# XiaokunSun/SemanticHuman

Hardware: AMD Instinct MI355X
Metric: training meshes/sec at 6890 verts, batch=64 (higher is better)
Workload: dtype f32

## Files before the change

semantichuman_amd/csrc/linear.hip:

```cpp
#include "sh_bf16.h"
#include "sh_adam.h"

#include <type_traits>

namespace {

constexpr int LT = 64;
constexpr int LK = 32;
constexpr int LTHREADS = 256;

struct SGParams {
    const float* a; long a_sm, a_sr;
    const float* b; long b_sn, b_sr;
    float* c; long c_sm, c_sn;
    const float* bias;
    float* slab;
    int M, N, R;
    int rchunk, nsplit, n_mtiles, n_ntiles;
    int a_mode, b_mode;
};

__device__ __forceinline__ void sg_load(const float* base, long s_row, long s_r, int mode, int row0, int nrows, int r0, int rend,
                                        int tid, f32x4 (&reg)[2], unsigned& mask) {
    mask = 0;
// ... 242 lines not shown
#pragma unroll
                for (int mt = 0; mt < MT; ++mt) acc[mt][nt] = __builtin_amdgcn_mfma_f32_16x16x4f32(w4[nt][t], x4[mt][t], acc[mt][nt], 0, 0, 0);
    };
    auto step = [&](int s, auto J) {
        constexpr int j = decltype(J)::value;
        load(s + LS_DEPTH - 1, xa[(j + LS_DEPTH - 1) % LS_DEPTH], wb[(j + LS_DEPTH - 1) % LS_DEPTH]);
        __builtin_amdgcn_sched_barrier(0);
        mma(xa[j], wb[j]);
    };
    if (nsteps > 0) {
#pragma unroll
        for (int d = 0; d < LS_DEPTH - 1; ++d) load(d, xa[d], wb[d]);
        for (int s = 0; s < nsteps; s += LS_DEPTH)
            if (ls_run_steps<0, LS_DEPTH>(s, nsteps, step)) break;
    }
#pragma unroll
    for (int mt = 0; mt < MT; ++mt) {
        const int m = 16 * mt + lr;
        if (m >= p.M) continue;
#pragma unroll
        for (int nt = 0; nt < 4; ++nt) {
            const int n = n0 + 16 * nt + 4 * kq;
            f32x4 v = acc[mt][nt];
            if (p.nsplit > 1) {
                *reinterpret_cast<f32x4*>(p.slab + ((long)sp * p.M + m) * p.N + n) = v;
            } else {
                if (p.bias) v += *reinterpret_cast<const f32x4*>(p.bias + n);
                *reinterpret_cast<f32x4*>(p.out + (long)m * p.N + n) = v;
            }
        }
    }
}

constexpr int LFD_STAGE = 40 * 1024, LFD_LDS = 3 * LFD_STAGE;
__device__ __forceinline__ f32x4 lin_x3_mma(const bf16x8 ah, const bf16x8 am, const bf16x8 al, const bf16x8 bh, const bf16x8 bm, const bf16x8 bl,
                                            f32x4 c) {
    c = __builtin_amdgcn_mfma_f32_16x16x32_bf16(al, bh, c, 0, 0, 0);
    c = __builtin_amdgcn_mfma_f32_16x16x32_bf16(ah, bl, c, 0, 0, 0);
    c = __builtin_amdgcn_mfma_f32_16x16x32_bf16(am, bm, c, 0, 0, 0);
    c = __builtin_amdgcn_mfma_f32_16x16x32_bf16(am, bh, c, 0, 0, 0);
    c = __builtin_amdgcn_mfma_f32_16x16x32_bf16(ah, bm, c, 0, 0, 0);
    return __builtin_amdgcn_mfma_f32_16x16x32_bf16(ah, bh, c, 0, 0, 0);
}
struct LinX3 { bf16x8 h, m, l; };
__device__ __forceinline__ LinX3 lin_split(const f32x4 a, const f32x4 b) {
    u32x4 h, m, l;
    sh_split3(a, b, h, m, l);
    return LinX3{__builtin_bit_cast(bf16x8, h), __builtin_bit_cast(bf16x8, m), __builtin_bit_cast(bf16x8, l)};
}

template <int MT, bool X3 = false>
__global__ __launch_bounds__(LTHREADS) void linear_fwd_dma_kernel(const LSParams p) {
    extern __shared__ __attribute__((aligned(16))) char smem[];
    const int lane = threadIdx.x & 63;
    const int wave = __builtin_amdgcn_readfirstlane((int)(threadIdx.x >> 6));
    const int item = sh_xcd_remap(blockIdx.x, gridDim.x) * 4 + wave;
    const int ng = item % p.groups, sp = item / p.groups;
    const int n0 = ng * 64, k_begin = sp * p.range;
    const int nst = (min(p.K, k_begin + p.range) - k_begin) >> 5;
    const int m_lo = 64 * (int)blockIdx.y, m_n = min(64, p.M - m_lo);
    const float* pa = p.a + (long)m_lo * p.K;
    const int lr = lane & 15, kq = lane >> 4;
    typedef __attribute__((address_space(3))) char* lptr_t;
    const unsigned lds0 = __builtin_amdgcn_readfirstlane((unsigned)(uintptr_t)(lptr_t)smem);
    auto dma16 = [](const void* gsrc, unsigned lds_dst) {
        asm volatile("s_mov_b32 m0, %1\n\ts_nop 0\n\tglobal_load_lds_dwordx4 %0, off" : : "v"(gsrc), "s"(lds_dst) : "memory", "m0");
    };
    const int drow = lane >> 3;
    const float* wsrc[8];
    const float* xsrc[2];
#pragma unroll
    for (int q = 0; q < 8; ++q) {
        const int r = 8 * q + drow, piece = (lane & 7) ^ ((r >> 1) & 7);
        wsrc[q] = p.w + (long)(n0 + r) * p.K + k_begin + 4 * piece;
    }
#pragma unroll
    for (int j = 0; j < 2; ++j) {
        const int r = 8 * (2 * wave + j) + drow, piece = (lane & 7) ^ ((r >> 1) & 7);
        xsrc[j] = pa + (long)min(r, m_n - 1) * p.K + k_begin + 4 * piece;
    }
    auto issue = [&](int st) {
        const unsigned slot = lds0 + (unsigned)((st % 3) * LFD_STAGE);
        const int off = 32 * (st < nst ? st : nst - 1);
#pragma unroll
        for (int j = 0; j < 2; ++j) dma16(xsrc[j] + off, slot + (unsigned)((2 * wave + j) * 1024));
#pragma unroll
        for (int q = 0; q < 8; ++q) dma16(wsrc[q] + off, slot + (unsigned)(8192 + wave * 8192 + q * 1024));
    };
    f32x4 acc[MT][4];
#pragma unroll
    for (int mt = 0; mt < MT; ++mt)
#pragma unroll
        for (int nt = 0; nt < 4; ++nt) acc[mt][nt] = (f32x4){0.f, 0.f, 0.f, 0.f};
    const int sw = (lr >> 1) & 7;
    const int foff0 = lr * 128 + ((kq ^ sw) << 4), foff1 = lr * 128 + (((4 + kq) ^ sw) << 4);
    if (nst > 0) {
        issue(0);
        issue(1);
        for (int st = 0; st < nst; ++st) {
            asm volatile("s_waitcnt vmcnt(10)" ::: "memory");
            __syncthreads();
            issue(st + 2);
            const char* sl = smem + (st % 3) * LFD_STAGE;
            const char* wl = sl + 8192 + wave * 8192;
            if constexpr (X3) {
                LinX3 xs[MT];
#pragma unroll
                for (int mt = 0; mt < MT; ++mt)
                    xs[mt] = lin_split(*reinterpret_cast<const f32x4*>(sl + mt * 2048 + foff0), *reinterpret_cast<const f32x4*>(sl + mt * 2048 + foff1));
#pragma unroll
                for (int nt = 0; nt < 4; ++nt) {
                    const LinX3 ws = lin_split(*reinterpret_cast<const f32x4*>(wl + nt * 2048 + foff0), *reinterpret_cast<const f32x4*>(wl + nt * 2048 + foff1));
#pragma unroll
                    for (int mt = 0; mt < MT; ++mt) acc[mt][nt] = lin_x3_mma(ws.h, ws.m, ws.l, xs[mt].h, xs[mt].m, xs[mt].l, acc[mt][nt]);
                }
                continue;
            }
#pragma unroll
            for (int h = 0; h < 2; ++h) {
                const int fo = h == 0 ? foff0 : foff1;
                f32x4 w4[4], x4[MT];
#pragma unroll
                for (int nt = 0; nt < 4; ++nt) w4[nt] = *reinterpret_cast<const f32x4*>(wl + nt * 2048 + fo);
#pragma unroll
                for (int mt = 0; mt < MT; ++mt) x4[mt] = *reinterpret_cast<const f32x4*>(sl + mt * 2048 + fo);
#pragma unroll
                for (int t = 0; t < 4; ++t)
#pragma unroll
                    for (int nt = 0; nt < 4; ++nt)
#pragma unroll
                        for (int mt = 0; mt < MT; ++mt) acc[mt][nt] = __builtin_amdgcn_mfma_f32_16x16x4f32(w4[nt][t], x4[mt][t], acc[mt][nt], 0, 0, 0);
            }
        }
        asm volatile("s_waitcnt vmcnt(0)" ::: "memory");
    }
#pragma unroll
    for (int mt = 0; mt < MT; ++mt) {
        if (16 * mt + lr >= m_n) continue;
        const int m = m_lo + 16 * mt + lr;
#pragma unroll
        for (int nt = 0; nt < 4; ++nt) {
            const int n = n0 + 16 * nt + 4 * kq;
            f32x4 v = acc[mt][nt];
            if (p.nsplit > 1) {
                *reinterpret_cast<f32x4*>(p.slab + ((long)sp * p.M + m) * p.N + n) = v;
            } else {
                if (p.bias) v += *reinterpret_cast<const f32x4*>(p.bias + n);
                *reinterpret_cast<f32x4*>(p.out + (long)m * p.N + n) = v;
            }
        }
    }
}

constexpr int LFW_WAVES = 8;
__global__ __launch_bounds__(LFW_WAVES * 64) void linear_fwd_wide_x3_kernel(const LSParams p) {
    extern __shared__ __attribute__((aligned(16))) char smem[];
    u32x4* Wl = reinterpret_cast<u32x4*>(smem);
    const int lane = threadIdx.x & 63, wave = sh_wave_id();
    const int n0 = sh_xcd_remap(blockIdx.x, gridDim.x) * 64;
    const int nks = p.K >> 5;
    const int lr = lane & 15, kq = lane >> 4;
    for (int f = wave; f < nks * 4; f += LFW_WAVES) {
        const int ks = f >> 2, nt = f & 3;
        const float* src = p.w + (long)(n0 + 16 * nt + lr) * p.K + 32 * ks + 8 * kq;
        u32x4 h, m, l;
        sh_split3(*reinterpret_cast<const f32x4*>(src), *reinterpret_cast<const f32x4*>(src + 4), h, m, l);
        u32x4* d = Wl + (long)f * 192 + lane;
        d[0] = h; d[64] = m; d[128] = l;
    }
    __syncthreads();
    for (int m0 = 16 * wave; m0 < p.M; m0 += 16 * LFW_WAVES) {
        const int mrow = m0 + lr;
        const float* xr = p.a + (long)min(mrow, p.M - 1) * p.K + 8 * kq;
        f32x4 acc[4];
#pragma unroll
        for (int nt = 0; nt < 4; ++nt) acc[nt] = (f32x4){0.f, 0.f, 0.f, 0.f};
        f32x4 xa = *reinterpret_cast<const f32x4*>(xr), xb = *reinterpret_cast<const f32x4*>(xr + 4);
        for (int ks = 0; ks < nks; ++ks) {
            const int kn = ks + 1 < nks ? ks + 1 : ks;
            const f32x4 na = *reinterpret_cast<const f32x4*>(xr + 32 * kn), nb = *reinterpret_cast<const f32x4*>(xr + 32 * kn + 4);
            const LinX3 xs = lin_split(xa, xb);
            const u32x4* wk = Wl + (long)ks * 4 * 192 + lane;
#pragma unroll
            for (int nt = 0; nt < 4; ++nt) {
                const u32x4 r0 = wk[nt * 192], r1 = wk[nt * 192 + 64], r2 = wk[nt * 192 + 128];
                acc[nt] = lin_x3_mma(__builtin_bit_cast(bf16x8, r0), __builtin_bit_cast(bf16x8, r1), __builtin_bit_cast(bf16x8, r2), xs.h, xs.m,
                                     xs.l, acc[nt]);
            }
            xa = na; xb = nb;
        }
        if (mrow < p.M) {
#pragma unroll
            for (int nt = 0; nt < 4; ++nt) {
                const int n = n0 + 16 * nt + 4 * kq;
                f32x4 v = acc[nt];
                if (p.bias) v += *reinterpret_cast<const f32x4*>(p.bias + n);
                *reinterpret_cast<f32x4*>(p.out + (long)mrow * p.N + n) = v;
            }
        }
    }
}

template <int MT>
__global__ __launch_bounds__(LTHREADS) void linear_bwd_data_stream_kernel(const LSParams p) {
    const int lane = threadIdx.x & 63, wave = sh_wave_id();
    const int item = sh_xcd_remap(blockIdx.x, gridDim.x) * 4 + wave;
    if (item >= p.groups * p.nsplit) return;
    const int kg = item % p.groups, sp = item / p.groups;
    const int k0 = kg * 64, n_begin = sp * p.range;
    const int nsteps = (min(p.N, n_begin + p.range) - n_begin) >> 4;
    const int la = lane & 15, rr = lane >> 4;
    const float* drow[MT];
#pragma unroll
    for (int mt = 0; mt < MT; ++mt) drow[mt] = p.a + (long)min(16 * mt + la, p.M - 1) * p.N + n_begin + 4 * rr;
    const float* wbase = p.w + (long)(n_begin + 4 * rr) * p.K + k0 + 4 * la;
    f32x4 dq[LS_DEPTH][MT], wq[LS_DEPTH][4], acc[4][MT];
#pragma unroll
    for (int t = 0; t < 4; ++t)
#pragma unroll
        for (int mt = 0; mt < MT; ++mt) acc[t][mt] = (f32x4){0.f, 0.f, 0.f, 0.f};
    auto load = [&](int s, f32x4 (&d4)[MT], f32x4 (&w4)[4]) {
        const int nb = 16 * (s < nsteps ? s : nsteps - 1);
#pragma unroll
        for (int mt = 0; mt < MT; ++mt) d4[mt] = *reinterpret_cast<const f32x4*>(drow[mt] + nb);
#pragma unroll
        for (int e = 0; e < 4; ++e) w4[e] = __builtin_nontemporal_load(reinterpret_cast<const f32x4*>(wbase + (long)(nb + e) * p.K));
    };
    auto mma = [&](const f32x4 (&d4)[MT], const f32x4 (&w4)[4]) {
#pragma unroll
        for (int e = 0; e < 4; ++e)
#pragma unroll
            for (int t = 0; t < 4; ++t)
#pragma unroll
                for (int mt = 0; mt < MT; ++mt) acc[t][mt] = __builtin_amdgcn_mfma_f32_16x16x4f32(w4[e][t], d4[mt][e], acc[t][mt], 0, 0, 0);
    };
    auto step = [&](int s, auto J) {
        constexpr int j = decltype(J)::value;
        load(s + LS_DEPTH - 1, dq[(j + LS_DEPTH - 1) % LS_DEPTH], wq[(j + LS_DEPTH - 1) % LS_DEPTH]);
        __builtin_amdgcn_sched_barrier(0);
        mma(dq[j], wq[j]);
    };
    if (nsteps > 0) {
#pragma unroll
        for (int d = 0; d < LS_DEPTH - 1; ++d) load(d, dq[d], wq[d]);
        for (int s = 0; s < nsteps; s += LS_DEPTH)
            if (ls_run_steps<0, LS_DEPTH>(s, nsteps, step)) break;
    }
#pragma unroll
    for (int mt = 0; mt < MT; ++mt) {
        const int m = 16 * mt + la;
        if (m >= p.M) continue;
        float* dst = (p.nsplit > 1 ? p.slab + ((long)sp * p.M + m) * p.K : p.out + (long)m * p.K) + k0 + 16 * rr;
#pragma unroll
        for (int jj = 0; jj < 4; ++jj)
            *reinterpret_cast<f32x4*>(dst + 4 * jj) = (f32x4){acc[0][mt][jj], acc[1][mt][jj], acc[2][mt][jj], acc[3][mt][jj]};
    }
}

template <int MT>
__global__ __launch_bounds__(LTHREADS) void linear_bwd_data_x3_kernel(const LSParams p) {
    const int lane = threadIdx.x & 63, wave = sh_wave_id();
    const int item = sh_xcd_remap(blockIdx.x, gridDim.x) * 4 + wave;
    if (item >= p.groups * p.nsplit) return;
    const int kg = item % p.groups, sp = item / p.groups;
    const int k0 = kg * 64, n_begin = sp * p.range;
    const int nsteps = (min(p.N, n_begin + p.range) - n_begin) >> 5;
    const int la = lane & 15, rr = lane >> 4;
    const float* drow[MT];
#pragma unroll
    for (int mt = 0; mt < MT; ++mt) drow[mt] = p.a + (long)min(16 * mt + la, p.M - 1) * p.N + n_begin + 4 * rr;
    const float* wbase = p.w + (long)(n_begin + 4 * rr) * p.K + k0 + 4 * la;
    f32x4 dq[2][MT][2], wq[2][8], acc[4][MT];
#pragma unroll
    for (int t = 0; t < 4; ++t)
#pragma unroll
        for (int mt = 0; mt < MT; ++mt) acc[t][mt] = (f32x4){0.f, 0.f, 0.f, 0.f};
    auto load = [&](int s, f32x4 (&d4)[MT][2], f32x4 (&w4)[8]) {
        const int nb = 32 * (s < nsteps ? s : nsteps - 1);
#pragma unroll
        for (int mt = 0; mt < MT; ++mt) {
            d4[mt][0] = *reinterpret_cast<const f32x4*>(drow[mt] + nb);
            d4[mt][1] = *reinterpret_cast<const f32x4*>(drow[mt] + nb + 16);
        }
#pragma unroll
        for (int j = 0; j < 8; ++j)
            w4[j] = __builtin_nontemporal_load(reinterpret_cast<const f32x4*>(wbase + (long)(nb + (j & 3) + 16 * (j >> 2)) * p.K));
    };
    auto mma = [&](const f32x4 (&d4)[MT][2], const f32x4 (&w4)[8]) {
        LinX3 ds[MT];
#pragma unroll
        for (int mt = 0; mt < MT; ++mt) ds[mt] = lin_split(d4[mt][0], d4[mt][1]);
#pragma unroll
        for (int t = 0; t < 4; ++t) {
            const LinX3 ws = lin_split((f32x4){w4[0][t], w4[1][t], w4[2][t], w4[3][t]}, (f32x4){w4[4][t], w4[5][t], w4[6][t], w4[7][t]});
#pragma unroll
            for (int mt = 0; mt < MT; ++mt) acc[t][mt] = lin_x3_mma(ws.h, ws.m, ws.l, ds[mt].h, ds[mt].m, ds[mt].l, acc[t][mt]);
        }
    };
    if (nsteps > 0) {
        load(0, dq[0], wq[0]);
        for (int s = 0; s < nsteps; s += 2) {
            load(s + 1, dq[1], wq[1]);
            __builtin_amdgcn_sched_barrier(0);
            mma(dq[0], wq[0]);
            if (s + 1 >= nsteps) break;
            load(s + 2, dq[0], wq[0]);
            __builtin_amdgcn_sched_barrier(0);
            mma(dq[1], wq[1]);
        }
    }
#pragma unroll
    for (int mt = 0; mt < MT; ++mt) {
        const int m = 16 * mt + la;
        if (m >= p.M) continue;
        float* dst = (p.nsplit > 1 ? p.slab + ((long)sp * p.M + m) * p.K : p.out + (long)m * p.K) + k0 + 16 * rr;
#pragma unroll
        for (int jj = 0; jj < 4; ++jj)
            *reinterpret_cast<f32x4*>(dst + 4 * jj) = (f32x4){acc[0][mt][jj], acc[1][mt][jj], acc[2][mt][jj], acc[3][mt][jj]};
    }
}

__global__ __launch_bounds__(LTHREADS) void linear_bwd_wgt_stream_kernel(const LSParams p) {
    const int lane = threadIdx.x & 63, wave = sh_wave_id();
    const int item = sh_xcd_remap(blockIdx.x, gridDim.x) * 4 + wave;
    const int ktiles = p.K >> 6;
    if (item >= (p.N >> 6) * ktiles) return;
    const int kt = item % ktiles, ntile = item / ktiles;
    const int n0 = ntile * 64, k0 = kt * 64;
    const int la = lane & 15, rr = lane >> 4;
    const int nsteps = (p.M + 3) >> 2;
    f32x4 acc[4][4];
#pragma unroll
    for (int a = 0; a < 4; ++a)
#pragma unroll
        for (int b = 0; b < 4; ++b) acc[a][b] = (f32x4){0.f, 0.f, 0.f, 0.f};
    f32x4 dq[4], xq[4];
    auto load = [&](int s, f32x4& d4, f32x4& x4) {
        s = s < nsteps ? s : nsteps - 1;
        const int m = 4 * s + rr;
        const int mc = m < p.M ? m : p.M - 1;
        d4 = *reinterpret_cast<const f32x4*>(p.a + (long)mc * p.N + n0 + 4 * la);
        x4 = *reinterpret_cast<const f32x4*>(p.w + (long)mc * p.K + k0 + 4 * la);
        if (m >= p.M) d4 = (f32x4){0.f, 0.f, 0.f, 0.f};
    };
    const bool own_bias = kt == 0 && p.dbias != nullptr;
    f32x4 bsum = {0.f, 0.f, 0.f, 0.f};
    auto mma = [&](const f32x4& d4, const f32x4& x4) {
#pragma unroll
        for (int tn = 0; tn < 4; ++tn)
#pragma unroll
            for (int tk = 0; tk < 4; ++tk) acc[tn][tk] = __builtin_amdgcn_mfma_f32_16x16x4f32(d4[tn], x4[tk], acc[tn][tk], 0, 0, 0);
        if (own_bias) bsum += d4;
    };
    load(0, dq[0], xq[0]); load(1, dq[1], xq[1]); load(2, dq[2], xq[2]);
    for (int s = 0; s < nsteps; s += 4) {
        load(s + 3, dq[3], xq[3]); __builtin_amdgcn_sched_barrier(0); mma(dq[0], xq[0]);
        if (s + 1 >= nsteps) break;
        load(s + 4, dq[0], xq[0]); __builtin_amdgcn_sched_barrier(0); mma(dq[1], xq[1]);
        if (s + 2 >= nsteps) break;
        load(s + 5, dq[1], xq[1]); __builtin_amdgcn_sched_barrier(0); mma(dq[2], xq[2]);
        if (s + 3 >= nsteps) break;
        load(s + 6, dq[2], xq[2]); __builtin_amdgcn_sched_barrier(0); mma(dq[3], xq[3]);
    }
    if (own_bias) {
#pragma unroll
        for (int j = 0; j < 4; ++j) {
            float v = bsum[j];
            v += __shfl_xor(v, 16, 64);
            v += __shfl_xor(v, 32, 64);
            bsum[j] = v;
        }
        if (rr == 0) *reinterpret_cast<f32x4*>(p.dbias + n0 + 4 * la) = bsum;
    }
#pragma unroll
    for (int tn = 0; tn < 4; ++tn)
#pragma unroll
        for (int jj = 0; jj < 4; ++jj) {
            float* dst = p.out + (long)(n0 + 16 * rr + 4 * jj + tn) * p.K + k0 + 4 * la;
            __builtin_nontemporal_store((f32x4){acc[tn][0][jj], acc[tn][1][jj], acc[tn][2][jj], acc[tn][3][jj]}, reinterpret_cast<f32x4*>(dst));
        }
}

constexpr int LWD_TILE = 16 * 1024, LWD_LDS = 5 * LWD_TILE;
template <bool X3 = false, bool ADAM = false, bool A16 = false, bool W16 = false>
__global__ __launch_bounds__(LTHREADS) __attribute__((amdgpu_waves_per_eu((X3 || ADAM) ? 2 : 1, (X3 || ADAM) ? 2 : 8)))
void linear_bwd_wgt_dma_kernel(const LSParams p) {
    extern __shared__ __attribute__((aligned(16))) char smem[];
    const int lane = threadIdx.x & 63;
    const int wave = __builtin_amdgcn_readfirstlane((int)(threadIdx.x >> 6));
    const int ktiles = p.K >> 6, kgroups = (ktiles + 3) >> 2;
    const int item = sh_xcd_remap(blockIdx.x, gridDim.x);
    const int kg = item % kgroups, ntile = item / kgroups;
    const int kt = kg * 4 + wave;
    const bool active = kt < ktiles;
    const int n0 = ntile * 64, k0 = (active ? kt : 0) * 64;
    const int la = lane & 15, rr = lane >> 4;
    const int nsteps = (p.M + 3) >> 2;
    typedef __attribute__((address_space(3))) char* lptr_t;
    const unsigned lds0 = __builtin_amdgcn_readfirstlane((unsigned)(uintptr_t)(lptr_t)smem);
    auto dma16 = [](const void* gsrc, unsigned lds_dst) {
        asm volatile("s_mov_b32 m0, %1\n\ts_nop 0\n\tglobal_load_lds_dwordx4 %0, off" : : "v"(gsrc), "s"(lds_dst) : "memory", "m0");
    };
    const int piece = (lane & 15) ^ ((lane >> 4) << 2);
    auto stage16 = [&](const __bf16* src, long ld, int col0, int row, int j, char* tile) {
        const bf16x8 v = *reinterpret_cast<const bf16x8*>(src + (long)min(row, p.M - 1) * ld + col0 + 8 * j);
        char* d = tile + (row >> 2) * 1024 + (row & 3) * 256;
        const int sw = (row & 3) << 2;
        *reinterpret_cast<f32x4*>(d + (((2 * j) ^ sw) << 4)) = (f32x4){(float)v[0], (float)v[1], (float)v[2], (float)v[3]};
        *reinterpret_cast<f32x4*>(d + (((2 * j + 1) ^ sw) << 4)) = (f32x4){(float)v[4], (float)v[5], (float)v[6], (float)v[7]};
    };
    if constexpr (A16) {
#pragma unroll
        for (int i = 0; i < 2; ++i) {
            const int q = 64 * i + lane;
            stage16(reinterpret_cast<const __bf16*>(p.a), p.N, n0, 16 * wave + (q >> 3), q & 7, smem);
        }
    } else {
#pragma unroll
    for (int i = 0; i < 4; ++i) {
        const int ins = 4 * wave + i, row = 4 * ins + (lane >> 4);
        dma16(p.a + (long)min(row, p.M - 1) * p.N + n0 + 4 * piece, lds0 + (unsigned)(ins * 1024));
    }
    }
    if constexpr (W16) {
#pragma unroll
        for (int i = 0; i < 8; ++i) {
            const int q = 64 * i + lane;
            stage16(reinterpret_cast<const __bf16*>(p.w), p.K, k0, q >> 3, q & 7, smem + (1 + wave) * LWD_TILE);
        }
    } else {
#pragma unroll
    for (int ins = 0; ins < 16; ++ins) {
        const int row = 4 * ins + (lane >> 4);
        dma16(p.w + (long)min(row, p.M - 1) * p.K + k0 + 4 * piece, lds0 + (unsigned)((1 + wave) * LWD_TILE + ins * 1024));
    }
    }
    float step_size = 0.f, bc2_sqrt = 1.f;
    if constexpr (ADAM) sh_adam_coeffs(p.ad.beta1, p.ad.beta2, p.ad.step[0], p.ad.lr[0], step_size, bc2_sqrt);
    asm volatile("s_waitcnt vmcnt(0)" ::: "memory");
    __syncthreads();
    if (!active) return;
    const char* ds = smem;
    const char* xs = smem + (1 + wave) * LWD_TILE;
    f32x4 acc[4][4];
#pragma unroll
    for (int a = 0; a < 4; ++a)
#pragma unroll
        for (int b = 0; b < 4; ++b) acc[a][b] = (f32x4){0.f, 0.f, 0.f, 0.f};
    const bool own_bias = kt == 0 && p.dbias != nullptr;
    f32x4 bsum = {0.f, 0.f, 0.f, 0.f};
    const int roff = rr * 256 + ((la ^ (rr << 2)) << 4);
    f32x4 apf[ADAM ? 2 : 1][4][3];
    auto adam_load = [&](int tn, int buf) {
#pragma unroll
        for (int jj = 0; jj < 4; ++jj) {
            const long o = (long)(n0 + 16 * rr + 4 * jj + tn) * p.K + k0 + 4 * la;
            apf[buf][jj][0] = __builtin_nontemporal_load(reinterpret_cast<const f32x4*>(p.out + o));
            apf[buf][jj][1] = __builtin_nontemporal_load(reinterpret_cast<const f32x4*>(p.am + o));
            apf[buf][jj][2] = __builtin_nontemporal_load(reinterpret_cast<const f32x4*>(p.av + o));
        }
    };
// ... 17 lines not shown
            for (int tn = 0; tn < 4; ++tn) {
                const LinX3 dn = lin_split((f32x4){d[0][tn], d[1][tn], d[2][tn], d[3][tn]}, (f32x4){d[4][tn], d[5][tn], d[6][tn], d[7][tn]});
#pragma unroll
                for (int tk = 0; tk < 4; ++tk) acc[tn][tk] = lin_x3_mma(dn.h, dn.m, dn.l, xk[tk].h, xk[tk].m, xk[tk].l, acc[tn][tk]);
            }
        }
    } else
    for (int s = 0; s < nsteps; ++s) {
        f32x4 d4 = *reinterpret_cast<const f32x4*>(ds + s * 1024 + roff);
        const f32x4 x4 = *reinterpret_cast<const f32x4*>(xs + s * 1024 + roff);
        if (4 * s + rr >= p.M) d4 = (f32x4){0.f, 0.f, 0.f, 0.f};
#pragma unroll
        for (int tn = 0; tn < 4; ++tn)
#pragma unroll
            for (int tk = 0; tk < 4; ++tk) acc[tn][tk] = __builtin_amdgcn_mfma_f32_16x16x4f32(d4[tn], x4[tk], acc[tn][tk], 0, 0, 0);
        if (own_bias) bsum += d4;
    }
    if (own_bias) {
#pragma unroll
        for (int j = 0; j < 4; ++j) {
            float v = bsum[j];
            v += __shfl_xor(v, 16, 64);
            v += __shfl_xor(v, 32, 64);
            bsum[j] = v;
        }
        if (rr == 0) *reinterpret_cast<f32x4*>(p.dbias + n0 + 4 * la) = bsum;
    }
    if constexpr (ADAM) {
#pragma unroll
        for (int tn = 0; tn < 4; ++tn) {
            if (tn + 1 < 4) adam_load(tn + 1, (tn + 1) & 1);
#pragma unroll
            for (int jj = 0; jj < 4; ++jj) {
                const long o = (long)(n0 + 16 * rr + 4 * jj + tn) * p.K + k0 + 4 * la;
                f32x4 pp = apf[tn & 1][jj][0], mm = apf[tn & 1][jj][1], vv = apf[tn & 1][jj][2];
#pragma unroll
                for (int tk = 0; tk < 4; ++tk) {
                    float p1 = pp[tk], m1 = mm[tk], v1 = vv[tk];
                    adam_update(p1, acc[tn][tk][jj], m1, v1, p.ad.w1, p.ad.b2, p.ad.w2, p.ad.eps, p.ad.wd, step_size, bc2_sqrt);
                    pp[tk] = p1; mm[tk] = m1; vv[tk] = v1;
                }
                *reinterpret_cast<f32x4*>(p.out + o) = pp;
                if (p.shadow) *reinterpret_cast<bf16x4*>(p.shadow + o) = sh_to_bf16x4(pp);
                __builtin_nontemporal_store(mm, reinterpret_cast<f32x4*>(p.am + o));
                __builtin_nontemporal_store(vv, reinterpret_cast<f32x4*>(p.av + o));
            }
        }
    } else {
#pragma unroll
    for (int tn = 0; tn < 4; ++tn)
#pragma unroll
        for (int jj = 0; jj < 4; ++jj) {
            float* dst = p.out + (long)(n0 + 16 * rr + 4 * jj + tn) * p.K + k0 + 4 * la;
            __builtin_nontemporal_store((f32x4){acc[tn][0][jj], acc[tn][1][jj], acc[tn][2][jj], acc[tn][3][jj]}, reinterpret_cast<f32x4*>(dst));
        }
    }
}

struct LSPlan { bool ok; int range, nsplit, groups; };
LSPlan plan_stream(int M, int out_cols, int red_len, int gran = 16, bool chunked = false) {
    LSPlan pl{false, red_len, 1, out_cols / 64};
    static const int on = sh_env_int("SH_LIN_STREAM", 1, 0, 1);
    static const int dma_on = sh_env_int("SH_LIN_DMA", 1, 0, 1);
    const bool big_ok = chunked && dma_on && red_len < 1024 && red_len % 32 == 0 && (out_cols / 64) % 4 == 0;
    if (!on || (M > 64 && !big_ok) || out_cols % 64 != 0 || red_len % gran != 0) return pl;
    pl.ok = true;
    static const int items = sh_env_int("SH_LIN_ITEMS", 1024, 64, 1 << 20);
    if (pl.groups < items / 2 && red_len >= 1024) {
        int ns = items / pl.groups;
        int rg = sh_cdiv(sh_cdiv(red_len, ns), gran) * gran;
        if (rg < 64) rg = 64;
        pl.range = rg;
        pl.nsplit = sh_cdiv(red_len, rg);
    }
    return pl;
}
bool aligned16(const void* a, const void* b, const void* c) {
    return ((reinterpret_cast<uintptr_t>(a) | reinterpret_cast<uintptr_t>(b) | reinterpret_cast<uintptr_t>(c)) & 15) == 0;
}

int mode_of(const float* base, long s_row, long s_r, int rows, int R) {
    const bool aligned = (reinterpret_cast<uintptr_t>(base) & 15) == 0;
    if (s_r == 1 && (s_row & 3) == 0 && (R & 3) == 0 && aligned) return 0;
    if (s_row == 1 && (s_r & 3) == 0 && (rows & 3) == 0 && aligned) return 1;
    return 2;
}

struct SGPlan { int nsplit, rchunk; };
SGPlan plan_split(int M, int N, int R) {
    const int tiles = sh_cdiv(M, LT) * sh_cdiv(N, LT);
    SGPlan pl{1, R};
    if (tiles < 512 && R >= 2048) {
        int ns = sh_cdiv(1024, tiles);
        int rc = sh_cdiv(sh_cdiv(R, ns), LK) * LK;
        if (rc < 256) rc = 256;
        pl.rchunk = rc;
        pl.nsplit = sh_cdiv(R, rc);
    }
    return pl;
}

int run_gemm(SGParams& p, void* ws, size_t ws_bytes, hipStream_t st, const char* what) {
    const SGPlan pl = plan_split(p.M, p.N, p.R);
    p.nsplit = pl.nsplit; p.rchunk = pl.rchunk;
    p.n_mtiles = sh_cdiv(p.M, LT); p.n_ntiles = sh_cdiv(p.N, LT);
    p.a_mode = mode_of(p.a, p.a_sm, p.a_sr, p.M, p.R);
    p.b_mode = mode_of(p.b, p.b_sn, p.b_sr, p.N, p.R);
    const float* bias = p.bias;
    if (p.nsplit > 1) {
        SH_REQUIRE(p.c_sn == 1 && p.c_sm == p.N, SH_ERR_UNSUPPORTED, "%s: split reduction needs a contiguous output", what);
        SH_REQUIRE(ws && ws_bytes >= (size_t)p.nsplit * p.M * p.N * sizeof(float), SH_ERR_WORKSPACE, "%s: workspace too small", what);
        p.slab = static_cast<float*>(ws);
        p.bias = nullptr;
    }
    const long grid = (long)p.n_mtiles * p.n_ntiles * p.nsplit;
    {
        ShProfScope ps(st, "skinny_gemm_kernel|%s M=%d N=%d R=%d split=%d modes=%d%d", what, p.M, p.N, p.R, p.nsplit, p.a_mode, p.b_mode);
        SH_LAUNCH_PS(ps, skinny_gemm_kernel, dim3((unsigned)grid), dim3(LTHREADS), 0, st, p);
    }
    if (p.nsplit > 1) {
        const long mn = (long)p.M * p.N;
        ShProfScope ps(st, "split_reduce_kernel");
        SH_LAUNCH_PS(ps, split_reduce_kernel, dim3((unsigned)((mn + 63) / 64)), dim3(1024), 0, st, p.slab, p.nsplit, mn, p.N,
                           bias, p.c);
    }
    SH_CHECK_LAUNCH(what);
    return SH_OK;
}

inline bool lin_x3(int mma_mode) {
    static const int on = sh_env_int("SH_LIN_X3", 1, 0, 1);
    return on && (mma_mode == SH_MMA_SPLIT3 || mma_mode == SH_MMA_PLANES3);
}

template <bool FWD>
int run_stream(LSParams& p, const LSPlan& pl, int cols, void* ws, size_t ws_bytes, hipStream_t st, const char* what, bool x3 = false) {
    p.range = pl.range; p.nsplit = pl.nsplit; p.groups = pl.groups;
    const float* bias = p.bias;
    if (p.nsplit > 1) {
        SH_REQUIRE(ws && ws_bytes >= (size_t)p.nsplit * p.M * cols * sizeof(float), SH_ERR_WORKSPACE, "%s: workspace too small", what);
        p.slab = static_cast<float*>(ws);
    }
    const int items = p.groups * p.nsplit, grid = sh_cdiv(items, 4), mchunks = sh_cdiv(p.M, 64), mt = p.M > 64 ? 4 : sh_cdiv(p.M, 16);
    SH_REQUIRE(mchunks == 1 || (FWD && p.nsplit == 1), SH_ERR_UNSUPPORTED, "%s: more than 64 rows need the unsplit forward form", what);
    {
        ShProfScope ps(st, "%s<%d>|M=%d N=%d K=%d split=%d", FWD ? "linear_fwd_stream_kernel" : "linear_bwd_data_stream_kernel", mt, p.M,
                       p.N, p.K, p.nsplit);
#define SH_LS_CASE(MTV)                                                                                                   \
    if (FWD) SH_LAUNCH_PS(ps, linear_fwd_stream_kernel<MTV>, dim3(grid), dim3(LTHREADS), 0, st, p);                     \
    else SH_LAUNCH_PS(ps, linear_bwd_data_stream_kernel<MTV>, dim3(grid), dim3(LTHREADS), 0, st, p)
        static const int dma_on = sh_env_int("SH_LIN_DMA", 1, 0, 1);
        const bool dma = FWD && dma_on && p.K % 32 == 0 && p.range % 32 == 0 && p.groups % 4 == 0;
        SH_REQUIRE(mchunks == 1 || dma, SH_ERR_UNSUPPORTED, "%s: more than 64 rows need the LDS-DMA forward form (SH_LIN_DMA=1)", what);
        if (x3 && !FWD) {
            snprintf(ps.name, sizeof ps.name, "linear_bwd_data_x3_kernel<%d>|M=%d N=%d K=%d split=%d", mt, p.M, p.N, p.K, p.nsplit);
            if (mt == 1) SH_LAUNCH_PS(ps, linear_bwd_data_x3_kernel<1>, dim3(grid), dim3(LTHREADS), 0, st, p);
            else if (mt == 2) SH_LAUNCH_PS(ps, linear_bwd_data_x3_kernel<2>, dim3(grid), dim3(LTHREADS), 0, st, p);
            else if (mt == 3) SH_LAUNCH_PS(ps, linear_bwd_data_x3_kernel<3>, dim3(grid), dim3(LTHREADS), 0, st, p);
            else SH_LAUNCH_PS(ps, linear_bwd_data_x3_kernel<4>, dim3(grid), dim3(LTHREADS), 0, st, p);
        } else if (x3 && dma) {
            static bool attr3_set = false;
            if (!attr3_set) {
                const void* ks[4] = {reinterpret_cast<const void*>(linear_fwd_dma_kernel<1, true>), reinterpret_cast<const void*>(linear_fwd_dma_kernel<2, true>),
                                     reinterpret_cast<const void*>(linear_fwd_dma_kernel<3, true>), reinterpret_cast<const void*>(linear_fwd_dma_kernel<4, true>)};
                for (const void* k : ks)
                    if (hipFuncSetAttribute(k, hipFuncAttributeMaxDynamicSharedMemorySize, 160 * 1024) != hipSuccess) {
                        (void)hipGetLastError();
                        sh_set_error("%s: cannot raise the dynamic LDS limit to %d bytes", what, LFD_LDS);
                        return SH_ERR_LAUNCH;
                    }
                attr3_set = true;
            }
            snprintf(ps.name, sizeof ps.name, "linear_fwd_x3_kernel<%d>|M=%d N=%d K=%d split=%d", mt, p.M, p.N, p.K, p.nsplit);
            if (mt == 1) SH_LAUNCH_PS(ps, (linear_fwd_dma_kernel<1, true>), dim3(grid, mchunks), dim3(LTHREADS), LFD_LDS, st, p);
            else if (mt == 2) SH_LAUNCH_PS(ps, (linear_fwd_dma_kernel<2, true>), dim3(grid, mchunks), dim3(LTHREADS), LFD_LDS, st, p);
            else if (mt == 3) SH_LAUNCH_PS(ps, (linear_fwd_dma_kernel<3, true>), dim3(grid, mchunks), dim3(LTHREADS), LFD_LDS, st, p);
            else SH_LAUNCH_PS(ps, (linear_fwd_dma_kernel<4, true>), dim3(grid, mchunks), dim3(LTHREADS), LFD_LDS, st, p);
        } else if (dma) {
            static bool attr_set = false;
            if (!attr_set) {
                const void* ks[4] = {reinterpret_cast<const void*>(linear_fwd_dma_kernel<1>), reinterpret_cast<const void*>(linear_fwd_dma_kernel<2>),
                                     reinterpret_cast<const void*>(linear_fwd_dma_kernel<3>), reinterpret_cast<const void*>(linear_fwd_dma_kernel<4>)};
                for (const void* k : ks)
                    if (hipFuncSetAttribute(k, hipFuncAttributeMaxDynamicSharedMemorySize, 160 * 1024) != hipSuccess) {
                        (void)hipGetLastError();
                        sh_set_error("%s: cannot raise the dynamic LDS limit to %d bytes", what, LFD_LDS);
                        return SH_ERR_LAUNCH;
                    }
                attr_set = true;
            }
            snprintf(ps.name, sizeof ps.name, "linear_fwd_dma_kernel<%d>|M=%d N=%d K=%d split=%d", mt, p.M, p.N, p.K, p.nsplit);
            if (mt == 1) SH_LAUNCH_PS(ps, linear_fwd_dma_kernel<1>, dim3(grid, mchunks), dim3(LTHREADS), LFD_LDS, st, p);
            else if (mt == 2) SH_LAUNCH_PS(ps, linear_fwd_dma_kernel<2>, dim3(grid, mchunks), dim3(LTHREADS), LFD_LDS, st, p);
            else if (mt == 3) SH_LAUNCH_PS(ps, linear_fwd_dma_kernel<3>, dim3(grid, mchunks), dim3(LTHREADS), LFD_LDS, st, p);
            else SH_LAUNCH_PS(ps, linear_fwd_dma_kernel<4>, dim3(grid, mchunks), dim3(LTHREADS), LFD_LDS, st, p);
        } else if (mt == 1) { SH_LS_CASE(1); } else if (mt == 2) { SH_LS_CASE(2); } else if (mt == 3) { SH_LS_CASE(3); } else { SH_LS_CASE(4); }
#undef SH_LS_CASE
    }
    if (p.nsplit > 1) {
        const long mn = (long)p.M * cols;
        ShProfScope ps(st, "split_reduce_kernel");
        SH_LAUNCH_PS(ps, split_reduce_kernel, dim3((unsigned)((mn + 63) / 64)), dim3(1024), 0, st, p.slab, p.nsplit, mn, cols, bias,
                           p.out);
    }
    SH_CHECK_LAUNCH(what);
    return SH_OK;
}

}


extern "C" {

size_t sh_linear_workspace(int M, int N, int K) {
    if (M <= 0 || N <= 0 || K <= 0) return 0;
    size_t need = 0;
    {
        for (int gran : {16, 32}) {
            const LSPlan f = plan_stream(M, N, K, gran), d = plan_stream(M, K, N, gran);
            if (f.ok && f.nsplit > 1 && (size_t)f.nsplit * M * N * sizeof(float) > need) need = (size_t)f.nsplit * M * N * sizeof(float);
            if (d.ok && d.nsplit > 1 && (size_t)d.nsplit * M * K * sizeof(float) > need) need = (size_t)d.nsplit * M * K * sizeof(float);
        }
    }
    const int dims[3][3] = {{M, N, K}, {M, K, N}, {N, K, M}};
    for (auto& d : dims) {
        const SGPlan pl = plan_split(d[0], d[1], d[2]);
        if (pl.nsplit > 1) {
            const size_t b = (size_t)pl.nsplit * d[0] * d[1] * sizeof(float);
            if (b > need) need = b;
        }
    }
    return need;
}

int sh_linear_fwd(const float* x, const float* weight, const float* bias, float* y, int M, int N, int K, void* workspace,
                  size_t workspace_bytes, int mma_mode, sh_stream_t stream) {
    SH_REQUIRE(x && weight && y && M > 0 && N > 0 && K > 0, SH_ERR_INVALID_ARG, "sh_linear_fwd: bad argument");
    SH_REQUIRE(sh_mma_mode_valid(mma_mode), SH_ERR_INVALID_ARG, "sh_linear_fwd: unknown mma_mode %d", mma_mode);
    if (lin_x3(mma_mode) && M > 64 && K % 32 == 0 && K <= 384 && N % 64 == 0 && aligned16(x, weight, y) &&
        (!bias || (reinterpret_cast<uintptr_t>(bias) & 15) == 0)) {
        static const int wide_on = sh_env_int("SH_LIN_WIDE", 1, 0, 1);
        if (wide_on) {
            hipStream_t st = static_cast<hipStream_t>(stream);
            const size_t smem = (size_t)(K / 32) * 4 * 3072;
            static bool attr_set = false;
            if (!attr_set) {
                if (hipFuncSetAttribute(reinterpret_cast<const void*>(linear_fwd_wide_x3_kernel), hipFuncAttributeMaxDynamicSharedMemorySize,
                                        160 * 1024) != hipSuccess) {
                    (void)hipGetLastError();
                    sh_set_error("linear_fwd: cannot raise the dynamic LDS limit to %zu bytes", smem);
                    return SH_ERR_LAUNCH;
                }
                attr_set = true;
            }
            LSParams s{};
            s.a = x; s.w = weight; s.bias = bias; s.out = y; s.M = M; s.N = N; s.K = K;
            ShProfScope ps(st, "linear_fwd_wide_x3_kernel|M=%d N=%d K=%d", M, N, K);
            SH_LAUNCH_PS(ps, linear_fwd_wide_x3_kernel, dim3(N / 64), dim3(LFW_WAVES * 64), smem, st, s);
            SH_CHECK_LAUNCH("linear_fwd_wide");
            return SH_OK;
        }
    }
    {
        const bool x3 = lin_x3(mma_mode) && K % 32 == 0 && (N / 64) % 4 == 0;
        static const int chunk_on = sh_env_int("SH_LIN_CHUNKED", 1, 0, 1);
        const LSPlan pl = plan_stream(M, N, K, x3 ? 32 : 16, chunk_on && M > 64);
        if (pl.ok && aligned16(x, weight, y) && (!bias || (reinterpret_cast<uintptr_t>(bias) & 15) == 0)) {
            LSParams s{};
            s.a = x; s.w = weight; s.bias = bias; s.out = y; s.M = M; s.N = N; s.K = K;
            return run_stream<true>(s, pl, N, workspace, workspace_bytes, static_cast<hipStream_t>(stream), "linear_fwd", x3);
        }
    }
    SGParams p{};
    p.a = x; p.a_sm = K; p.a_sr = 1;
    p.b = weight; p.b_sn = K; p.b_sr = 1;
    p.c = y; p.c_sm = N; p.c_sn = 1; p.bias = bias;
    p.M = M; p.N = N; p.R = K;
    return run_gemm(p, workspace, workspace_bytes, static_cast<hipStream_t>(stream), "linear_fwd");
}

int sh_linear_bwd_data(const float* dy, const float* weight, float* dx, int M, int N, int K, void* workspace,
                       size_t workspace_bytes, int mma_mode, sh_stream_t stream) {
    SH_REQUIRE(dy && weight && dx && M > 0 && N > 0 && K > 0, SH_ERR_INVALID_ARG, "sh_linear_bwd_data: bad argument");
    SH_REQUIRE(sh_mma_mode_valid(mma_mode), SH_ERR_INVALID_ARG, "sh_linear_bwd_data: unknown mma_mode %d", mma_mode);
    {
        const bool x3 = lin_x3(mma_mode) && N % 32 == 0;
        const LSPlan pl = plan_stream(M, K, N, x3 ? 32 : 16);
        if (pl.ok && aligned16(dy, weight, dx)) {
            LSParams s{};
            s.a = dy; s.w = weight; s.bias = nullptr; s.out = dx; s.M = M; s.N = N; s.K = K;
            return run_stream<false>(s, pl, K, workspace, workspace_bytes, static_cast<hipStream_t>(stream), "linear_bwd_data", x3);
        }
    }
    SGParams p{};
    p.a = dy; p.a_sm = N; p.a_sr = 1;
    p.b = weight; p.b_sn = 1; p.b_sr = K;
    p.c = dx; p.c_sm = K; p.c_sn = 1; p.bias = nullptr;
    p.M = M; p.N = K; p.R = N;
    return run_gemm(p, workspace, workspace_bytes, static_cast<hipStream_t>(stream), "linear_bwd_data");
}

static bool wgt_dma_attr() {
    static bool attr_set = false;
    if (!attr_set) {
        for (const void* k : {reinterpret_cast<const void*>(linear_bwd_wgt_dma_kernel<false>), reinterpret_cast<const void*>(linear_bwd_wgt_dma_kernel<true>),
                              reinterpret_cast<const void*>(linear_bwd_wgt_dma_kernel<false, true>), reinterpret_cast<const void*>(linear_bwd_wgt_dma_kernel<true, true>),
                              reinterpret_cast<const void*>(linear_bwd_wgt_dma_kernel<false, true, true, false>),
// ... 105 lines not shown
```

Before: 46600.

## Share activation bf16x3 splits through LDS in x3 forward and backward-data linears

Adds two new x3 (three-way bf16 split) linear kernels. In each, the activation operand is split once per block and stored in shared memory instead of every wave splitting it again. The forward variant uses two waves per 64-column group, each covering half the columns, with a 3-stage LDS-DMA pipeline and double-buffered activation fragments. The backward-data variant pre-splits the activation rows in chunks of 8 steps into LDS. Both are on by default behind env switches and aim to remove redundant split arithmetic, at the cost of more LDS, extra barriers and possible occupancy loss.

```diff
diff --git a/semantichuman_amd/csrc/linear.hip b/semantichuman_amd/csrc/linear.hip
--- a/semantichuman_amd/csrc/linear.hip
+++ b/semantichuman_amd/csrc/linear.hip
@@ -418,6 +418,101 @@
     }
 }
 
+constexpr int LFS_THREADS = 512, LFS_FRAGS = 12 * 1024, LFS_LDS = LFD_LDS + 2 * LFS_FRAGS;
+template <int MT>
+__global__ __launch_bounds__(LFS_THREADS) void linear_fwd_x3s_kernel(const LSParams p) {
+    extern __shared__ __attribute__((aligned(16))) char smem[];
+    const int lane = threadIdx.x & 63;
+    const int wave = __builtin_amdgcn_readfirstlane((int)(threadIdx.x >> 6));
+    const int g = wave >> 1, hf = wave & 1;
+    const int item = sh_xcd_remap(blockIdx.x, gridDim.x) * 4 + g;
+    const int ng = item % p.groups, sp = item / p.groups;
+    const int n0 = ng * 64, k_begin = sp * p.range;
+    const int nst = (min(p.K, k_begin + p.range) - k_begin) >> 5;
+    const int m_lo = 64 * (int)blockIdx.y, m_n = min(64, p.M - m_lo);
+    const float* pa = p.a + (long)m_lo * p.K;
+    const int lr = lane & 15, kq = lane >> 4;
+    typedef __attribute__((address_space(3))) char* lptr_t;
+    const unsigned lds0 = __builtin_amdgcn_readfirstlane((unsigned)(uintptr_t)(lptr_t)smem);
+    auto dma16 = [](const void* gsrc, unsigned lds_dst) {
+        asm volatile("s_mov_b32 m0, %1\n\ts_nop 0\n\tglobal_load_lds_dwordx4 %0, off" : : "v"(gsrc), "s"(lds_dst) : "memory", "m0");
+    };
+    const int drow = lane >> 3;
+    const float* wsrc[4];
+#pragma unroll
+    for (int q = 0; q < 4; ++q) {
+        const int r = 8 * (4 * hf + q) + drow, piece = (lane & 7) ^ ((r >> 1) & 7);
+        wsrc[q] = p.w + (long)(n0 + r) * p.K + k_begin + 4 * piece;
+    }
+    const float* xsrc = pa + (long)min(16 * g + lr, m_n - 1) * p.K + k_begin + 4 * (4 * hf + kq);
+    auto issue = [&](int st) {
+        const unsigned slot = lds0 + (unsigned)((st % 3) * LFD_STAGE);
+        const int off = 32 * (st < nst ? st : nst - 1);
+        dma16(xsrc + off, slot + (unsigned)(wave * 1024));
+#pragma unroll
+        for (int q = 0; q < 4; ++q) dma16(wsrc[q] + off, slot + (unsigned)(8192 + g * 8192 + (4 * hf + q) * 1024));
+    };
+    auto xsplit = [&](int st) {
+        asm volatile("s_waitcnt vmcnt(9)" ::: "memory");
+        const f32x4 raw = *reinterpret_cast<const f32x4*>(smem + (st % 3) * LFD_STAGE + wave * 1024 + lane * 16);
+        u32x2 h, m, l;
+        sh_split3_quad(raw, h, m, l);
+        char* d = smem + LFD_LDS + (st & 1) * LFS_FRAGS + g * 3072 + lane * 16 + hf * 8;
+        *reinterpret_cast<u32x2*>(d) = h;
+        *reinterpret_cast<u32x2*>(d + 1024) = m;
+        *reinterpret_cast<u32x2*>(d + 2048) = l;
+    };
+    f32x4 acc[MT][2];
+#pragma unroll
+    for (int mt = 0; mt < MT; ++mt)
+#pragma unroll
+        for (int n2 = 0; n2 < 2; ++n2) acc[mt][n2] = (f32x4){0.f, 0.f, 0.f, 0.f};
+    const int sw = (lr >> 1) & 7;
+    const int foff0 = lr * 128 + ((kq ^ sw) << 4), foff1 = lr * 128 + (((4 + kq) ^ sw) << 4);
+    if (nst > 0) {
+        issue(0);
+        issue(1);
+        if (g < MT) xsplit(0);
+        for (int st = 0; st < nst; ++st) {
+            asm volatile("s_waitcnt vmcnt(5)" ::: "memory");
+            __syncthreads();
+            issue(st + 2);
+            const char* wl = smem + (st % 3) * LFD_STAGE + 8192 + g * 8192 + hf * 4096;
+            const char* xf = smem + LFD_LDS + (st & 1) * LFS_FRAGS + lane * 16;
+            LinX3 xs[MT];
+#pragma unroll
+            for (int mt = 0; mt < MT; ++mt)
+                xs[mt] = LinX3{__builtin_bit_cast(bf16x8, *reinterpret_cast<const u32x4*>(xf + mt * 3072)),
+                               __builtin_bit_cast(bf16x8, *reinterpret_cast<const u32x4*>(xf + mt * 3072 + 1024)),
+                               __builtin_bit_cast(bf16x8, *reinterpret_cast<const u32x4*>(xf + mt * 3072 + 2048))};
+#pragma unroll
+            for (int n2 = 0; n2 < 2; ++n2) {
+                const LinX3 ws = lin_split(*reinterpret_cast<const f32x4*>(wl + n2 * 2048 + foff0), *reinterpret_cast<const f32x4*>(wl + n2 * 2048 + foff1));
+#pragma unroll
+                for (int mt = 0; mt < MT; ++mt) acc[mt][n2] = lin_x3_mma(ws.h, ws.m, ws.l, xs[mt].h, xs[mt].m, xs[mt].l, acc[mt][n2]);
+                if (n2 == 0 && g < MT && st + 1 < nst) xsplit(st + 1);
+            }
+        }
+        asm volatile("s_waitcnt vmcnt(0)" ::: "memory");
+    }
+#pragma unroll
+    for (int mt = 0; mt < MT; ++mt) {
+        if (16 * mt + lr >= m_n) continue;
+        const int m = m_lo + 16 * mt + lr;
+#pragma unroll
+        for (int n2 = 0; n2 < 2; ++n2) {
+            const int n = n0 + 32 * hf + 16 * n2 + 4 * kq;
+            f32x4 v = acc[mt][n2];
+            if (p.nsplit > 1) {
+                *reinterpret_cast<f32x4*>(p.slab + ((long)sp * p.M + m) * p.N + n) = v;
+            } else {
+                if (p.bias) v += *reinterpret_cast<const f32x4*>(p.bias + n);
+                *reinterpret_cast<f32x4*>(p.out + (long)m * p.N + n) = v;
+            }
+        }
+    }
+}
+
 constexpr int LFW_WAVES = 8;
 __global__ __launch_bounds__(LFW_WAVES * 64) void linear_fwd_wide_x3_kernel(const LSParams p) {
     extern __shared__ __attribute__((aligned(16))) char smem[];
@@ -573,6 +668,91 @@
             load(s + 2, dq[0], wq[0]);
             __builtin_amdgcn_sched_barrier(0);
             mma(dq[1], wq[1]);
+        }
+    }
+#pragma unroll
+    for (int mt = 0; mt < MT; ++mt) {
+        const int m = 16 * mt + la;
+        if (m >= p.M) continue;
+        float* dst = (p.nsplit > 1 ? p.slab + ((long)sp * p.M + m) * p.K : p.out + (long)m * p.K) + k0 + 16 * rr;
+#pragma unroll
+        for (int jj = 0; jj < 4; ++jj)
+            *reinterpret_cast<f32x4*>(dst + 4 * jj) = (f32x4){acc[0][mt][jj], acc[1][mt][jj], acc[2][mt][jj], acc[3][mt][jj]};
+    }
+}
+
+constexpr int LBS_CHUNK = 8, LBS_LDS = LBS_CHUNK * 12 * 1024;
+template <int MT>
+__global__ __launch_bounds__(LTHREADS) void linear_bwd_data_x3s_kernel(const LSParams p) {
+    extern __shared__ __attribute__((aligned(16))) char smem[];
+    const int lane = threadIdx.x & 63;
+    const int wave = __builtin_amdgcn_readfirstlane((int)(threadIdx.x >> 6));
+    const int item = sh_xcd_remap(blockIdx.x, gridDim.x) * 4 + wave;
+    const int kg = item % p.groups, sp = item / p.groups;
+    const int k0 = kg * 64, n_begin = sp * p.range;
+    const int nsteps = (min(p.N, n_begin + p.range) - n_begin) >> 5;
+    const int la = lane & 15, rr = lane >> 4;
+    const float* drow = p.a + (long)min(16 * wave + la, p.M - 1) * p.N + n_begin + 4 * rr;
+    const float* wbase = p.w + (long)(n_begin + 4 * rr) * p.K + k0 + 4 * la;
+    f32x4 wq[2][8], acc[4][MT];
+#pragma unroll
+    for (int t = 0; t < 4; ++t)
+#pragma unroll
+        for (int mt = 0; mt < MT; ++mt) acc[t][mt] = (f32x4){0.f, 0.f, 0.f, 0.f};
+    auto load = [&](int s, f32x4 (&w4)[8]) {
+        const int nb = 32 * (s < nsteps ? s : nsteps - 1);
+#pragma unroll
+        for (int j = 0; j < 8; ++j)
+            w4[j] = __builtin_nontemporal_load(reinterpret_cast<const f32x4*>(wbase + (long)(nb + (j & 3) + 16 * (j >> 2)) * p.K));
+    };
+    auto presplit = [&](int s0) {
+        if (s0 > 0) __syncthreads();
+        if (wave < MT) {
+            f32x4 d4[LBS_CHUNK][2];
+#pragma unroll
+            for (int c = 0; c < LBS_CHUNK; ++c) {
+                const int nb = 32 * min(s0 + c, nsteps - 1);
+                d4[c][0] = *reinterpret_cast<const f32x4*>(drow + nb);
+                d4[c][1] = *reinterpret_cast<const f32x4*>(drow + nb + 16);
+            }
+            if (s0 == 0) load(0, wq[0]);
+            __builtin_amdgcn_sched_barrier(0);
+#pragma unroll
+            for (int c = 0; c < LBS_CHUNK; ++c) {
+                u32x4 h, m, l;
+                sh_split3(d4[c][0], d4[c][1], h, m, l);
+                u32x4* d = reinterpret_cast<u32x4*>(smem + (c * MT + wave) * 3072) + lane;
+                d[0] = h; d[64] = m; d[128] = l;
+            }
+        } else if (s0 == 0) {
+            load(0, wq[0]);
+        }
+        __syncthreads();
+    };
+    auto mma = [&](int s, const f32x4 (&w4)[8]) {
+        const u32x4* df = reinterpret_cast<const u32x4*>(smem + (s & (LBS_CHUNK - 1)) * MT * 3072) + lane;
+        LinX3 ds[MT];
+#pragma unroll
+        for (int mt = 0; mt < MT; ++mt)
+            ds[mt] = LinX3{__builtin_bit_cast(bf16x8, df[mt * 192]), __builtin_bit_cast(bf16x8, df[mt * 192 + 64]),
+                           __builtin_bit_cast(bf16x8, df[mt * 192 + 128])};
+#pragma unroll
+        for (int t = 0; t < 4; ++t) {
+            const LinX3 ws = lin_split((f32x4){w4[0][t], w4[1][t], w4[2][t], w4[3][t]}, (f32x4){w4[4][t], w4[5][t], w4[6][t], w4[7][t]});
+#pragma unroll
+            for (int mt = 0; mt < MT; ++mt) acc[t][mt] = lin_x3_mma(ws.h, ws.m, ws.l, ds[mt].h, ds[mt].m, ds[mt].l, acc[t][mt]);
+        }
+    };
+    if (nsteps > 0) {
+        for (int s = 0; s < nsteps; s += 2) {
+            if ((s & (LBS_CHUNK - 1)) == 0) presplit(s);
+            load(s + 1, wq[1]);
+            __builtin_amdgcn_sched_barrier(0);
+            mma(s, wq[0]);
+            if (s + 1 >= nsteps) break;
+            load(s + 2, wq[0]);
+            __builtin_amdgcn_sched_barrier(0);
+            mma(s + 1, wq[1]);
         }
     }
 #pragma unroll
@@ -896,7 +1076,44 @@
         static const int dma_on = sh_env_int("SH_LIN_DMA", 1, 0, 1);
         const bool dma = FWD && dma_on && p.K % 32 == 0 && p.range % 32 == 0 && p.groups % 4 == 0;
         SH_REQUIRE(mchunks == 1 || dma, SH_ERR_UNSUPPORTED, "%s: more than 64 rows need the LDS-DMA forward form (SH_LIN_DMA=1)", what);
-        if (x3 && !FWD) {
+        static const int fwd_shared = sh_env_int("SH_LIN_FWD_SHARED", 1, 0, 1), bwd_shared = sh_env_int("SH_LIN_BWD_SHARED", 1, 0, 1);
+        if (x3 && !FWD && bwd_shared && p.groups % 4 == 0) {
+            static bool attrb_set = false;
+            if (!attrb_set) {
+                const void* ks[4] = {reinterpret_cast<const void*>(linear_bwd_data_x3s_kernel<1>), reinterpret_cast<const void*>(linear_bwd_data_x3s_kernel<2>),
+                                     reinterpret_cast<const void*>(linear_bwd_data_x3s_kernel<3>), reinterpret_cast<const void*>(linear_bwd_data_x3s_kernel<4>)};
+                for (const void* k : ks)
+                    if (hipFuncSetAttribute(k, hipFuncAttributeMaxDynamicSharedMemorySize, 160 * 1024) != hipSuccess) {
+                        (void)hipGetLastError();
+                        sh_set_error("%s: cannot raise the dynamic LDS limit to %d bytes", what, LBS_LDS);
+                        return SH_ERR_LAUNCH;
+                    }
+                attrb_set = true;
+            }
+            snprintf(ps.name, sizeof ps.name, "linear_bwd_data_x3_kernel<%d>|M=%d N=%d K=%d split=%d", mt, p.M, p.N, p.K, p.nsplit);
+            if (mt == 1) SH_LAUNCH_PS(ps, linear_bwd_data_x3s_kernel<1>, dim3(grid), dim3(LTHREADS), LBS_LDS, st, p);
+            else if (mt == 2) SH_LAUNCH_PS(ps, linear_bwd_data_x3s_kernel<2>, dim3(grid), dim3(LTHREADS), LBS_LDS, st, p);
+            else if (mt == 3) SH_LAUNCH_PS(ps, linear_bwd_data_x3s_kernel<3>, dim3(grid), dim3(LTHREADS), LBS_LDS, st, p);
+            else SH_LAUNCH_PS(ps, linear_bwd_data_x3s_kernel<4>, dim3(grid), dim3(LTHREADS), LBS_LDS, st, p);
+        } else if (x3 && dma && fwd_shared) {
+            static bool attrs_set = false;
+            if (!attrs_set) {
+                const void* ks[4] = {reinterpret_cast<const void*>(linear_fwd_x3s_kernel<1>), reinterpret_cast<const void*>(linear_fwd_x3s_kernel<2>),
+                                     reinterpret_cast<const void*>(linear_fwd_x3s_kernel<3>), reinterpret_cast<const void*>(linear_fwd_x3s_kernel<4>)};
+                for (const void* k : ks)
+                    if (hipFuncSetAttribute(k, hipFuncAttributeMaxDynamicSharedMemorySize, 160 * 1024) != hipSuccess) {
+                        (void)hipGetLastError();
+                        sh_set_error("%s: cannot raise the dynamic LDS limit to %d bytes", what, LFS_LDS);
+                        return SH_ERR_LAUNCH;
+                    }
+                attrs_set = true;
+            }
+            snprintf(ps.name, sizeof ps.name, "linear_fwd_x3_kernel<%d>|M=%d N=%d K=%d split=%d", mt, p.M, p.N, p.K, p.nsplit);
+            if (mt == 1) SH_LAUNCH_PS(ps, linear_fwd_x3s_kernel<1>, dim3(grid, mchunks), dim3(LFS_THREADS), LFS_LDS, st, p);
+            else if (mt == 2) SH_LAUNCH_PS(ps, linear_fwd_x3s_kernel<2>, dim3(grid, mchunks), dim3(LFS_THREADS), LFS_LDS, st, p);
+            else if (mt == 3) SH_LAUNCH_PS(ps, linear_fwd_x3s_kernel<3>, dim3(grid, mchunks), dim3(LFS_THREADS), LFS_LDS, st, p);
+            else SH_LAUNCH_PS(ps, linear_fwd_x3s_kernel<4>, dim3(grid, mchunks), dim3(LFS_THREADS), LFS_LDS, st, p);
+        } else if (x3 && !FWD) {
             snprintf(ps.name, sizeof ps.name, "linear_bwd_data_x3_kernel<%d>|M=%d N=%d K=%d split=%d", mt, p.M, p.N, p.K, p.nsplit);
             if (mt == 1) SH_LAUNCH_PS(ps, linear_bwd_data_x3_kernel<1>, dim3(grid), dim3(LTHREADS), 0, st, p);
             else if (mt == 2) SH_LAUNCH_PS(ps, linear_bwd_data_x3_kernel<2>, dim3(grid), dim3(LTHREADS), 0, st, p);
```

New measurement: 46750, median of 6. Within noise of the previous version (+0.3%).
